# Merricx/zksnake

Measured on AMD Instinct MI355X. Metric: BN254 G1 MSM throughput, higher is better.
Workload: dtype u32 limbs (254-bit modular integers)

## Files before the change

### zksnake_amd/csrc/host.hip

```cpp
#include <dirent.h>
#include <unistd.h>
#include <cstring>
#include <map>
#include <mutex>
#include <vector>
#include "common.hip.h"
#include "codec.hip.h"

extern "C" void zk_ntt_free_cache(void);
extern "C" void zk_msm_free_all(void);
extern "C" void zk_ntt_stream_released(void* stream);

namespace zkmi {

static std::mutex g_cache_mutex;
static std::multimap<size_t, void*> g_cache_free;
static std::map<void*, size_t> g_cache_live;
static size_t g_cache_bytes = 0;
static const size_t CACHE_BUDGET = 6ull << 30;
static const size_t CACHE_MAX_BLOCK = 2ull << 30;

int dev_alloc_cached(void** p, size_t bytes) {
    if (bytes == 0) bytes = 1;
    {
        std::lock_guard<std::mutex> lock(g_cache_mutex);
        auto it = g_cache_free.find(bytes);
        if (it != g_cache_free.end()) {
            *p = it->second;
            g_cache_free.erase(it);
            g_cache_bytes -= bytes;
            g_cache_live[*p] = bytes;
            return ZK_OK;
        }
    }
    hipError_t e = hipMalloc(p, bytes);
    if (e != hipSuccess) {
        dev_cache_release();
        e = hipMalloc(p, bytes);
    }
    if (e != hipSuccess) return fail(ZK_ERR_HIP, std::string("hipMalloc(") + std::to_string(bytes) + " bytes): " + hipGetErrorString(e));
    std::lock_guard<std::mutex> lock(g_cache_mutex);
    g_cache_live[*p] = bytes;
    return ZK_OK;
}

void dev_free_cached(void* p) {
    if (!p) return;
    size_t bytes = 0;
    {
        std::lock_guard<std::mutex> lock(g_cache_mutex);
        auto it = g_cache_live.find(p);
        if (it != g_cache_live.end()) {
            bytes = it->second;
            g_cache_live.erase(it);
            if (bytes <= CACHE_MAX_BLOCK && g_cache_bytes + bytes <= CACHE_BUDGET) {
                g_cache_free.emplace(bytes, p);
                g_cache_bytes += bytes;
                return;
            }
        }
    }
    (void)hipFree(p);
}

static std::vector<hipStream_t> g_stream_pool[2];
static std::multimap<size_t, void*> g_pinned_free;
static std::map<void*, size_t> g_pinned_live;

void dev_cache_release() {
    std::lock_guard<std::mutex> lock(g_cache_mutex);
    for (auto& kv : g_cache_free) (void)hipFree(kv.second);
    g_cache_free.clear();
    g_cache_bytes = 0;
    for (auto& pool : g_stream_pool) {
        for (hipStream_t st : pool) (void)hipStreamDestroy(st);
        pool.clear();
    }
    for (auto& kv : g_pinned_free) (void)hipHostFree(kv.second);
    g_pinned_free.clear();
}

int stream_acquire(bool high_priority, hipStream_t* out) {
    {
        std::lock_guard<std::mutex> lock(g_cache_mutex);
        auto& pool = g_stream_pool[high_priority ? 1 : 0];
        if (!pool.empty()) {
            *out = pool.back();
            pool.pop_back();
            return ZK_OK;
        }
    }
    int lo = 0, hi = 0;
    ZK_HIP(hipDeviceGetStreamPriorityRange(&lo, &hi));
    ZK_HIP(hipStreamCreateWithPriority(out, hipStreamDefault, high_priority ? hi : lo));
    return ZK_OK;
}

void stream_release(bool high_priority, hipStream_t st) {
    if (!st) return;
    std::lock_guard<std::mutex> lock(g_cache_mutex);
    auto& pool = g_stream_pool[high_priority ? 1 : 0];
    if (pool.size() < 32) pool.push_back(st);
    else (void)hipStreamDestroy(st);
}

int pinned_alloc_cached(void** p, size_t bytes) {
    {
        std::lock_guard<std::mutex> lock(g_cache_mutex);
        auto it = g_pinned_free.find(bytes);
        if (it != g_pinned_free.end()) {
            *p = it->second;
            g_pinned_free.erase(it);
            g_pinned_live[*p] = bytes;
            return ZK_OK;
        }
    }
    ZK_HIP(hipHostMalloc(p, bytes));
    std::lock_guard<std::mutex> lock(g_cache_mutex);
    g_pinned_live[*p] = bytes;
    return ZK_OK;
}

void pinned_free_cached(void* p) {
    if (!p) return;
    std::lock_guard<std::mutex> lock(g_cache_mutex);
    auto it = g_pinned_live.find(p);
    if (it != g_pinned_live.end() && g_pinned_free.size() < 64 && it->second <= (1u << 20)) {
        g_pinned_free.emplace(it->second, p);
        g_pinned_live.erase(it);
        return;
    }
    if (it != g_pinned_live.end()) g_pinned_live.erase(it);
    (void)hipHostFree(p);
}


template <class G>
static Affine<typename G::F> load_point(const uint64_t* src) {
    typedef typename G::F F;
    const uint32_t* w = reinterpret_cast<const uint32_t*>(src);
    Affine<F> p;
    p.x = F::from_canonical(w);
    p.y = F::from_canonical(w + F::LIMBS);
    return p;
}

template <class G>
static void store_point(uint64_t* dst, const Affine<typename G::F>& p) {
    typedef typename G::F F;
    uint32_t* w = reinterpret_cast<uint32_t*>(dst);
    F::to_canonical(w, p.x);
    F::to_canonical(w + F::LIMBS, p.y);
}

template <class G>
static Affine<typename G::HostF> load_point64(const uint64_t* src) {
    typedef typename G::HostF HF;
    const uint32_t* w = reinterpret_cast<const uint32_t*>(src);
    return {HF::from_canonical(w), HF::from_canonical(w + HF::LIMBS)};
}
template <class G>
static void store_point64(uint64_t* dst, const Affine<typename G::HostF>& p) {
    G::HostF::affine_to_canonical(p, dst);
}

template <class G>
static bool point_on_curve(const Affine<typename G::F>& p) {
    typedef typename G::F F;
    typename F::T b = F::from_canonical(CurveConsts<G>::b());
    return aff_on_curve<F>(p, b);
}

template <class FrP>
static void reduce_scalar(uint32_t* k, const uint64_t* scalar) {
    memcpy(k, scalar, FrP::W * 4);
    for (int r = 0; r < 10; ++r) {
        uint32_t t[FrP::W];
        if (fp_sub_mod_raw<FrP>(t, k)) break;
        memcpy(k, t, sizeof(t));
    }
}


template <class G>
static int compress_impl(const uint64_t* a, uint8_t* out) {
    int code = point_encode<G>(reinterpret_cast<const uint32_t*>(a), out);
    return code ? fail(ZK_ERR_POINT, codec_message(code)) : ZK_OK;
}

template <class G>
static int decompress_impl(const uint8_t* in, uint64_t* out) {
    int code = point_decode<G>(in, reinterpret_cast<uint32_t*>(out));
    return code ? fail(ZK_ERR_POINT, codec_message(code)) : ZK_OK;
}


template <class P>
static Fp<P> fr_root(uint64_t n) {
    int log_n = log2_u64(n);
    Fp<P> w = fp_const<P>(P::ROOT);
    for (int k = 0; k < P::TWO_ADICITY - log_n; ++k) w = fp_sqr<P>(w);
    return w;
}

template <class P>
static int lagrange_impl(uint64_t n_in, const uint64_t* tau_c, uint64_t* out) {
    uint64_t n = next_pow2_u64(n_in == 0 ? 1 : n_in);
    int log_n = log2_u64(n);
    if (log_n > P::TWO_ADICITY) return fail(ZK_ERR_DOMAIN, "Domain size is too large");
    Fp<P> tau = fp_from_canonical<P>(reinterpret_cast<const uint32_t*>(tau_c));
    Fp<P> w = fr_root<P>(n);
    Fp<P> tn = tau;
    for (int k = 0; k < log_n; ++k) tn = fp_sqr<P>(tn);
    Fp<P> z = fp_sub<P>(tn, fp_one<P>());
    uint32_t* o = reinterpret_cast<uint32_t*>(out);
    if (fp_is_zero<P>(z)) {
        Fp<P> cur = fp_one<P>();
        for (uint64_t i = 0; i < n; ++i) {
            Fp<P> v = fp_eq<P>(cur, tau) ? fp_one<P>() : fp_zero<P>();
            fp_to_canonical<P>(o + i * P::W, v);
            cur = fp_mul<P>(cur, w);
        }
        return ZK_OK;
    }
    uint32_t nn[P::W] = {0};
    nn[0] = (uint32_t)n;
    nn[1] = (uint32_t)(n >> 32);
    Fp<P> zn = fp_mul<P>(z, fp_inv<P>(fp_from_canonical<P>(nn)));
    std::vector<Fp<P>> den(n), pre(n), wi(n);
    Fp<P> cur = fp_one<P>(), run = fp_one<P>();
    for (uint64_t i = 0; i < n; ++i) {
        wi[i] = cur;
        den[i] = fp_sub<P>(tau, cur);
        pre[i] = run;
        run = fp_mul<P>(run, den[i]);
        cur = fp_mul<P>(cur, w);
    }
    Fp<P> inv = fp_inv<P>(run);
    for (uint64_t i = n; i-- > 0;) {
        Fp<P> di = fp_mul<P>(inv, pre[i]);
        inv = fp_mul<P>(inv, den[i]);
        Fp<P> l = fp_mul<P>(fp_mul<P>(zn, wi[i]), di);
        fp_to_canonical<P>(o + i * P::W, l);
    }
    return ZK_OK;
}

template <class P>
static int poly_eval_impl(uint64_t n, const uint64_t* coeffs, const uint64_t* x_c, uint64_t* out) {
    const uint32_t* c = reinterpret_cast<const uint32_t*>(coeffs);
    Fp<P> x = fp_from_canonical<P>(reinterpret_cast<const uint32_t*>(x_c));
    Fp<P> acc = fp_zero<P>();
    for (uint64_t i = n; i-- > 0;) acc = fp_add<P>(fp_mul<P>(acc, x), fp_from_canonical<P>(c + i * P::W));
    fp_to_canonical<P>(reinterpret_cast<uint32_t*>(out), acc);
    return ZK_OK;
}

template <class P>
static int poly_div_linear_impl(uint64_t n, const uint64_t* coeffs, const uint64_t* root_c, uint64_t* q, uint64_t* rem) {
    const uint32_t* c = reinterpret_cast<const uint32_t*>(coeffs);
    uint32_t* qo = reinterpret_cast<uint32_t*>(q);
    Fp<P> root = fp_from_canonical<P>(reinterpret_cast<const uint32_t*>(root_c));
    Fp<P> carry = fp_zero<P>();
    for (uint64_t i = n; i-- > 1;) {
        carry = fp_add<P>(fp_from_canonical<P>(c + i * P::W), fp_mul<P>(carry, root));
        fp_to_canonical<P>(qo + (i - 1) * P::W, carry);
    }
    Fp<P> r0 = n ? fp_add<P>(fp_from_canonical<P>(c), fp_mul<P>(carry, root)) : fp_zero<P>();
    fp_to_canonical<P>(reinterpret_cast<uint32_t*>(rem), r0);
    return ZK_OK;
}

template <class P>
static int grand_product_impl(uint64_t n, const uint64_t* num, const uint64_t* den, uint64_t* out) {
    const uint32_t* a = reinterpret_cast<const uint32_t*>(num);
    const uint32_t* b = reinterpret_cast<const uint32_t*>(den);
    uint32_t* o = reinterpret_cast<uint32_t*>(out);
    std::vector<Fp<P>> d(n), pre(n);
    Fp<P> run = fp_one<P>();
    for (uint64_t i = 0; i < n; ++i) {
        d[i] = fp_from_canonical<P>(b + i * P::W);
        if (fp_is_zero<P>(d[i])) return fail(ZK_ERR_ARG, "grand product: zero denominator");
        pre[i] = run;
        run = fp_mul<P>(run, d[i]);
    }
    Fp<P> inv = fp_inv<P>(run);
    for (uint64_t i = n; i-- > 0;) {
        Fp<P> di = fp_mul<P>(inv, pre[i]);
        inv = fp_mul<P>(inv, d[i]);
        d[i] = di;
    }
    Fp<P> acc = fp_one<P>();
    fp_to_canonical<P>(o, acc);
    for (uint64_t i = 0; i < n; ++i) {
        acc = fp_mul<P>(fp_mul<P>(acc, fp_from_canonical<P>(a + i * P::W)), d[i]);
        fp_to_canonical<P>(o + (i + 1) * P::W, acc);
    }
    return ZK_OK;
}

template <class P>
static int scale_add_impl(uint64_t n, uint64_t* acc, const uint64_t* x, const uint64_t* s_c) {
    uint32_t* a = reinterpret_cast<uint32_t*>(acc);
    const uint32_t* xs = reinterpret_cast<const uint32_t*>(x);
    Fp<P> s = fp_from_canonical<P>(reinterpret_cast<const uint32_t*>(s_c));
    for (uint64_t i = 0; i < n; ++i) {
        Fp<P> v = fp_add<P>(fp_from_canonical<P>(a + i * P::W), fp_mul<P>(s, fp_from_canonical<P>(xs + i * P::W)));
        fp_to_canonical<P>(a + i * P::W, v);
    }
    return ZK_OK;
}

static int g_device = -1;

constexpr int ZK_WANT_HW_QUEUES = 12;
static std::mutex g_queue_mu;
static int g_queue_status = -1, g_queue_count = 0;

static bool hip_runtime_started() {
    if (const char* t = getenv("ZKMI_TEST_RUNTIME_STARTED")) return atoi(t) != 0;
    DIR* d = opendir("/proc/self/fd");
    if (!d) return false;
    bool found = false;
    char path[64], target[256];
    while (struct dirent* e = readdir(d)) {
        if (e->d_name[0] == '.') continue;
        snprintf(path, sizeof(path), "/proc/self/fd/%s", e->d_name);
        const ssize_t k = readlink(path, target, sizeof(target) - 1);
        if (k <= 0) continue;
        target[k] = 0;
        if (strcmp(target, "/dev/kfd") == 0) { found = true; break; }
    }
    closedir(d);
    return found;
}

static int hw_queues_prepare(int* queues) {
    std::lock_guard<std::mutex> lock(g_queue_mu);
    if (g_queue_status < 0) {
        const bool started = hip_runtime_started();
        const char* env = getenv("GPU_MAX_HW_QUEUES");
        if (env && *env) {
            g_queue_count = atoi(env);
            const char* ours = getenv("ZKMI_HW_QUEUES_SET_BY_LIBRARY");
            g_queue_status = (ours && *ours == '1' && g_queue_count == ZK_WANT_HW_QUEUES) ? ZK_QUEUES_SET_BY_LIBRARY : ZK_QUEUES_CALLER;
        } else if (!started) {
            char v[16];
            snprintf(v, sizeof(v), "%d", ZK_WANT_HW_QUEUES);
            setenv("GPU_MAX_HW_QUEUES", v, 0);
            setenv("ZKMI_HW_QUEUES_SET_BY_LIBRARY", "1", 1);
            g_queue_count = ZK_WANT_HW_QUEUES;
            g_queue_status = ZK_QUEUES_SET_BY_LIBRARY;
        } else {
            g_queue_count = 0;
            g_queue_status = ZK_QUEUES_TOO_LATE;
        }
    }
    if (queues) *queues = g_queue_count;
    return g_queue_status;
}

__global__ void spin_kernel(uint64_t ticks) {
    const uint64_t t0 = wall_clock64();
    while (wall_clock64() - t0 < ticks) {}
}

}

using namespace zkmi;

extern "C" {

int zk_device_count(void) {
    int n = 0;
    if (hipGetDeviceCount(&n) != hipSuccess) return 0;
    return n;
}

int zk_hw_queues_prepare(int* queues) { return hw_queues_prepare(queues); }

int zk_init(int device) {
    (void)hw_queues_prepare(nullptr);
    int n = zk_device_count();
    if (n <= 0) return fail(ZK_ERR_HIP, "no HIP device visible: libzkmi has no CPU fallback");
    if (device < 0 || device >= n) return fail(ZK_ERR_ARG, "device index out of range");
    ZK_HIP(hipSetDevice(device));
    g_device = device;
    return ZK_OK;
}

int zk_init_ex(int device, int* queue_status, int* queues) {
    const int st = hw_queues_prepare(queues);
    if (queue_status) *queue_status = st;
    return zk_init(device);
}

int zk_debug_spin_dev(void* stream, uint64_t microseconds) {
    hipLaunchKernelGGL(spin_kernel, dim3(1), dim3(64), 0, (hipStream_t)stream, microseconds * 100ull);
    ZK_HIP(hipGetLastError());
    return ZK_OK;
}

int zk_shutdown(void) {
    zk_msm_free_all();
    zk_ntt_free_cache();
    dev_cache_release();
    return ZK_OK;
}

int zk_dev_alloc(uint64_t bytes, void** d_ptr) {
    return dev_alloc_cached(d_ptr, bytes ? bytes : 1);
}
int zk_dev_free(void* d_ptr) {
    ZK_HIP(hipDeviceSynchronize());
    dev_free_cached(d_ptr);
    return ZK_OK;
}
int zk_dev_upload(void* d_dst, const void* h_src, uint64_t bytes) {
    if (bytes) ZK_HIP(hipMemcpy(d_dst, h_src, bytes, hipMemcpyHostToDevice));
    return ZK_OK;
// ... 189 lines not shown
```

### zksnake_amd/csrc/msm_impl.hip.h

```cpp
#pragma once
#include <algorithm>
#include <chrono>
#include <memory>
#include <vector>
#include "common.hip.h"
#include "msm_plan.h"
#include "pair.hip.h"
#include "setup_impl.hip.h"
#include "codec.hip.h"
#include "glv_params.h"

#include "msm_common.hip.h"
#include "msm_accumulate.hip.h"
#include "msm_reduce.hip.h"
#include "msm_host_tail.h"

namespace zkmi {
using mem::DevBuf;

#if defined(ZK_GROUP) && (!defined(ZK_PART) || ZK_PART == 0)
extern template __global__ void accumulate_kernel<ZK_GROUP>(const uint32_t*, const uint32_t*, const uint32_t*, const uint32_t*, uint32_t, uint32_t, uint32_t, uint32_t*, uint32_t*);
extern template __global__ void accumulate_split_kernel<ZK_GROUP>(const uint32_t*, const uint32_t*, const uint32_t*, const uint32_t*, uint32_t, uint32_t, uint32_t, uint32_t*, uint32_t*);
extern template __global__ void bases_to_mont_kernel<ZK_GROUP>(const uint32_t*, uint64_t, uint32_t*, int);
extern template __global__ void combine_kernel<ZK_GROUP>(const uint32_t*, const uint32_t*, uint32_t, uint32_t, const uint32_t*, const uint32_t*, uint32_t*);
extern template __global__ void strided_sum_kernel<ZK_GROUP>(const uint32_t*, uint32_t*, SumJob, SumJob, uint32_t);
extern template __global__ void weighted_sum_kernel<ZK_GROUP>(const uint32_t*, uint32_t, uint32_t, const uint32_t*, uint32_t, uint32_t*);
ZK_SETUP_EXTERN_TEMPLATES(ZK_GROUP)
ZK_CODEC_EXTERN_TEMPLATES(ZK_GROUP)
#endif

#if !defined(ZK_PART) || ZK_PART == 0

template <class G>
static int precompute_table(uint32_t* table, uint64_t n, int c, int w_first, int w_count) {
    typedef typename G::F F;
    constexpr int AW = 2 * F::LIMBS, XW = 4 * F::LIMBS;
    if (w_first == 0 && w_count == 1) return ZK_OK;
    DevBuf temp_buf;
    ZK_HIP_RC(temp_buf.alloc(n * XW * 4));
    uint32_t* const temp = temp_buf.as();
    const unsigned blocks = (unsigned)((n + 255) / 256);
    const unsigned nblocks = (unsigned)((n + (uint64_t)NORM_THREADS * NORM_E - 1) / ((uint64_t)NORM_THREADS * NORM_E));
    hipLaunchKernelGGL(dbl_rows_kernel<G>, dim3(blocks), dim3(256), 0, 0, temp, n, c * w_first, (const uint32_t*)table);
    if (w_first > 0) hipLaunchKernelGGL(normalize_kernel<G>, dim3(nblocks), dim3(NORM_THREADS), 0, 0, temp, n, table, 0);
    for (int k = 1; k < w_count; ++k) {
        hipLaunchKernelGGL(dbl_rows_kernel<G>, dim3(blocks), dim3(256), 0, 0, temp, n, c, (const uint32_t*)nullptr);
        hipLaunchKernelGGL(normalize_kernel<G>, dim3(nblocks), dim3(NORM_THREADS), 0, 0, temp, n, table + (size_t)k * n * AW, 0);
    }
    ZK_HIP(hipGetLastError());
    ZK_HIP(hipDeviceSynchronize());
    return ZK_OK;
}

template <class G>
struct FixedTable {
    std::vector<uint64_t> base;
    DevBuf d_table;
    int nwin = 0;
    std::mutex mu;
    static FixedTable& get() {
        static FixedTable* const t = new FixedTable();
        return *t;
    }
    void release() {
        std::lock_guard<std::mutex> lock(mu);
        d_table.reset();
        base.clear();
    }
    int ensure(const uint64_t* base_limbs) {
        typedef typename G::F F;
        typedef typename G::Fr FrP;
        constexpr int AW = 2 * F::LIMBS, XW = 4 * F::LIMBS;
        const size_t words64 = AW / 2;
        if (d_table && base.size() == words64 && memcmp(base.data(), base_limbs, words64 * 8) == 0) return ZK_OK;
        d_table.reset();
        base.clear();
        nwin = (FrP::BITS + 1 + FIXED_C - 1) / FIXED_C;
        std::vector<uint32_t> wb((size_t)nwin * AW);
        {
            const uint32_t* w = reinterpret_cast<const uint32_t*>(base_limbs);
            Affine<F> g = {F::from_canonical(w), F::from_canonical(w + F::LIMBS)};
            XYZZ<F> acc = xyzz_from_affine<F>(g);
            for (int j = 0; j < nwin; ++j) {
                Affine<F> a = xyzz_to_affine<F>(acc);
                F::store(wb.data() + (size_t)j * AW, a.x);
                F::store(wb.data() + (size_t)j * AW + F::LIMBS, a.y);
                if (j + 1 < nwin) for (int k = 0; k < FIXED_C; ++k) acc = xyzz_dbl<F>(acc);
            }
        }
        const uint64_t rows = (uint64_t)nwin * FIXED_HALF;
        DevBuf table, d_wb, temp;
        ZK_HIP_RC(table.alloc(rows * AW * 4));
        ZK_HIP_RC(d_wb.alloc(wb.size() * 4));
        ZK_HIP_RC(temp.alloc(rows * XW * 4));
        ZK_HIP(hipMemcpy(d_wb.as(), wb.data(), wb.size() * 4, hipMemcpyHostToDevice));
        hipLaunchKernelGGL(fixed_table_kernel<G>, dim3((unsigned)((rows + 255) / 256)), dim3(256), 0, 0, d_wb.as(), nwin, temp.as());
        hipLaunchKernelGGL(normalize_kernel<G>, dim3((unsigned)((rows + (uint64_t)NORM_THREADS * NORM_E - 1) / ((uint64_t)NORM_THREADS * NORM_E))),
                           dim3(NORM_THREADS), 0, 0, temp.as(), rows, table.as(), 0);
        ZK_HIP(hipGetLastError());
        ZK_HIP(hipDeviceSynchronize());
        d_table = std::move(table);
        base.assign(base_limbs, base_limbs + words64);
        return ZK_OK;
    }
};

template <class G>
struct MsmPlan : MsmPlanBase {
    typedef typename G::F F;
    typedef typename G::Fr FrP;
    static constexpr int AW = 2 * F::LIMBS;
    static constexpr int XW = 4 * F::LIMBS;
    static constexpr uint64_t SEG_TARGET_LANES = 256ull * 1024;
    static constexpr int MAX_C = 20;
    bool wide = false;
    enum class Phase { All, SortOnly, Rest };
    enum class Run { Idle, Sorted, Pending };

    struct Work {
        DevBuf partials, buckets, rows, fin;
        DevBuf parts;
        hipEvent_t ev_acc0 = nullptr, ev_accs = nullptr, ev_acc1 = nullptr;
        bool acc_from_accs = false;
        hipEvent_t ev_release = nullptr;
        bool lent = false;
        uint32_t seg_len = 0;
        int w_first = 0, w_count = 0;
        uint32_t groups = 0;
    };

    uint64_t n = 0;
    uint64_t n_api = 0;
    bool glv = false;
    bool pre = false;
    int pw_first = 0, pw_count = 0;
    ReduceShape shape;
    Work ws;
    MsmFront front;
    std::shared_ptr<DevBuf> bases_block;
    uint32_t* d_bases = nullptr;
    uint32_t* h_final = nullptr;
    hipEvent_t ev_start = nullptr, ev_end = nullptr;

    ~MsmPlan() override {
        (void)hipDeviceSynchronize();
        pinned_free_cached(h_final);
        for (hipEvent_t e : {ws.ev_acc0, ws.ev_accs, ws.ev_acc1, ws.ev_release, ev_start, ev_end}) if (e) (void)hipEventDestroy(e);
        stream_release((create_flags & ZK_MSM_HIGH_PRIORITY) != 0, own_stream);
    }

    int init(uint64_t n_points, const void* bases, int bases_on_device, int flags, int window_bits, int win_first, int win_count,
             const MsmPlan* share = nullptr) {
        const bool trace = opt.trace_init;
        auto t_prev = std::chrono::steady_clock::now();
        auto mark = [&](const char* what) {
            if (!trace) return;
            auto now = std::chrono::steady_clock::now();
            fprintf(stderr, "[plan init] %-24s %8.1f us\n", what, std::chrono::duration<double, std::micro>(now - t_prev).count());
            t_prev = now;
        };
        create_flags = flags;
        seg_lanes_at_init = opt.segment_lanes ? opt.segment_lanes : SEG_TARGET_LANES;
        pre = (flags & ZK_MSM_PRECOMPUTE) != 0;
        if (n_points == 0 || n_points > (1ull << 26)) return fail(ZK_ERR_ARG, "MSM size must be in [1, 2^26]");
        const MsmLayout lay = msm_layout(FrP::BITS, GlvOf<G>::OK, n_points, flags, window_bits, win_count <= 0);
        glv = share ? share->glv : lay.glv;
        n_api = n_points;
        n = glv ? 2 * n_points : n_points;
        entries_per_window = n;
        c = lay.c;
        if (c < 2 || c > MAX_C) return fail(ZK_ERR_ARG, "window bits must be in [2, 20]");
        if (c > 16 && !pre) return fail(ZK_ERR_ARG, "windows wider than 16 bits need a fixed-base plan (ZK_MSM_PRECOMPUTE)");
        wide = c > 16;
        nwin = glv ? glv_window_count(c) : window_count(FrP::BITS + 1, c);
        if (win_count <= 0) { win_first = 0; win_count = nwin; }
        if (win_first < 0 || win_first + win_count > nwin) return fail(ZK_ERR_ARG, "window range out of bounds");
        pw_first = win_first;
        pw_count = win_count;
        if (!reduce_shape(c, wide, &shape)) return fail(ZK_ERR_ARG, "window too wide for the reduction stage");
        const uint64_t entries = (uint64_t)pw_count * n;
        if (entries > 0x7FFFFFFFull) return fail(ZK_ERR_ARG, "MSM too large");

        ZK_HIP_RC(stream_acquire((flags & ZK_MSM_HIGH_PRIORITY) != 0, &own_stream));
        if (share) {
            bases_block = share->bases_block;
            d_bases = share->d_bases;
        } else {
            bases_block = std::make_shared<DevBuf>();
            ZK_HIP_RC(bases_block->alloc((pre ? (uint64_t)pw_count : 1ull) * n * AW * 4));
            d_bases = bases_block->as();
            if (bases_on_device) {
                launch_bases_to_mont<G>((const uint32_t*)bases, n_api, d_bases, glv ? 1 : 0, nullptr);
            } else {
                DevBuf tmp;
                ZK_HIP_RC(tmp.alloc(n_api * AW * 4));
                ZK_HIP(hipMemcpy(tmp.as(), bases, n_api * AW * 4, hipMemcpyHostToDevice));
                launch_bases_to_mont<G>(tmp.as(), n_api, d_bases, glv ? 1 : 0, nullptr);
                ZK_HIP(hipDeviceSynchronize());
            }
            ZK_HIP(hipGetLastError());
            if (pre) {
                int rc = precompute_table<G>(d_bases, n, c, pw_first, pw_count);
                if (rc) return rc;
            }
        }
        mark("stream + bases");
        {
            FrontLayout fl;
            fl.c = c; fl.B = shape.B; fl.n = n; fl.n_api = n_api; fl.pre = pre; fl.wide = wide; fl.glv = glv ? &GlvOf<G>::P::K : nullptr;
            fl.pw_first = pw_first; fl.pw_count = pw_count; fl.nwin = nwin; fl.curve = G::CURVE;
            ZK_HIP_RC(front.init(fl, &opt));
        }
        const uint64_t max_sets = pre ? 1ull : (uint64_t)pw_count;
        ZK_HIP_RC(pinned_alloc_cached((void**)&h_final, (size_t)max_sets * shape.blocks() * 2 * XW * 4));
        mark("scalars/digits/pinned");
        ZK_HIP(hipEventCreateWithFlags(&ev_start, hipEventDisableSystemFence));
        ZK_HIP(hipEventCreate(&ev_end));
        {
            const uint64_t keys = max_sets * shape.B;
            const uint32_t seg_full = pick_seg_len(entries);
            const uint64_t max_segs = std::max<uint64_t>(entries / seg_full, std::min<uint64_t>(entries / 8, seg_lanes_at_init)) + keys + 8;
            ZK_HIP_RC(front.alloc_workspace());
            ZK_HIP_RC(ws.partials.alloc(max_segs * XW * 4));
            ZK_HIP_RC(ws.buckets.alloc(keys * XW * 4));
            ZK_HIP_RC(ws.rows.alloc(max_sets * (shape.R + shape.C) * XW * 4));
            if (reduce_parts_per_set(shape)) ZK_HIP_RC(ws.parts.alloc(max_sets * reduce_parts_per_set(shape) * XW * 4));
            ZK_HIP_RC(ws.fin.alloc(max_sets * shape.blocks() * 2 * XW * 4));
            for (hipEvent_t* e : {&ws.ev_acc0, &ws.ev_accs, &ws.ev_acc1, &ws.ev_release}) ZK_HIP(hipEventCreate(e));
        }
        mark("workspace + events");
        ZK_HIP_RC(front.set_kernel_attributes());
        ZK_HIP(weighted_sum_set_attributes<G>());
        mark("func attributes");
        ZK_HIP(hipDeviceSynchronize());
        mark("device sync");
        return ZK_OK;
    }

    uint32_t pick_seg_len(uint64_t entries) const {
        const uint64_t target = opt.segment_lanes ? opt.segment_lanes : SEG_TARGET_LANES;
        uint64_t sl = (entries + target - 1) / target;
        if (sl < 8) sl = 8;
        if (sl > 64) sl = 64;
        if (pre) {
            uint64_t per_bucket = entries / shape.B;
            uint64_t want = (per_bucket + 11) / 12;
            if (want > sl) sl = want;
            if (sl > 1024) sl = 1024;
        }
        return (uint32_t)sl;
    }


    bool split_pairs_on() const {
        if constexpr (AccumulateSplit<G>::ON) return opt.split_pairs < 0 ? AccumulateSplit<G>::DEFAULT : opt.split_pairs != 0;
        return false;
    }

    int stage_accumulate(uint32_t m, const SortedView& sv, hipStream_t st, bool prio_steps) {
        Work& l = ws;
        const uint32_t n_keys = l.groups * shape.B;
        const uint64_t lanes_needed = ((uint64_t)l.w_count * m + sv.seg_len - 1) / sv.seg_len;
        launch_accumulate<G>(split_pairs_on(), lanes_needed, d_bases, sv.sorted, sv.bstart, sv.sstart, n_keys, sv.seg_len, prio_steps ? 1u : 0u,
                             l.partials.as(), l.buckets.as(), st);
        ZK_HIP(hipEventRecord(l.ev_acc1, st));
        launch_combine<G>(l.partials.as(), sv.sstart, n_keys, sv.big_list, sv.big_count, l.buckets.as(), st);
        ZK_HIP(hipGetLastError());
        return ZK_OK;
    }

    int stage_reduce(hipStream_t st) {
        Work& l = ws;
        const uint32_t groups = l.groups;
        const ReducePlan plan = reduce_plan(shape, groups, opt.sum_one_step, opt.lanes_per_output);
        uint32_t* const row_sums = l.rows.as();
        const uint32_t* in = l.buckets.as();
        for (int k = 0; k < plan.steps; ++k) {
            uint32_t* const out = k + 1 < plan.steps ? l.parts.as() : row_sums;
            launch_strided_sum<G>(in, out, plan.step[k].rows, plan.step[k].cols, plan.step[k].lpo, st);
            in = out;
        }
        launch_weighted_sum<G>(row_sums, shape.R, groups, row_sums + (size_t)groups * shape.R * XW, shape.C, l.fin.as(), st);
        ZK_HIP(hipGetLastError());
        ZK_HIP(hipMemcpyAsync(h_final, l.fin.as(), (size_t)groups * shape.blocks() * 2 * XW * 4, hipMemcpyDeviceToHost, st));
        return ZK_OK;
    }

    int run_stages(uint32_t m, uint32_t dstride, hipStream_t st, const SortExport* borrowed = nullptr, Phase phase = Phase::All, hipEvent_t gate = nullptr) {
        Work& l = ws;
        int rc;
        const uint32_t seg_len = borrowed ? borrowed->view.seg_len : (phase == Phase::Rest ? l.seg_len : pick_seg_len((uint64_t)l.w_count * m));
        l.seg_len = seg_len;
        if (phase == Phase::Rest) {
        } else if (borrowed) {
            ZK_HIP(hipStreamWaitEvent(st, borrowed->sorted_ready, 0));
        } else if ((rc = front.sort(m, dstride, seg_len, l.w_first, l.w_count, l.groups, st))) {
            return rc;
        }
        const SortedView sv = borrowed ? borrowed->view : front.view();
        if (phase != Phase::Rest) ZK_HIP(hipEventRecord(l.ev_acc0, st));
        if (phase == Phase::SortOnly) return ZK_OK;
        if (gate) ZK_HIP(hipStreamWaitEvent(st, gate, 0));
        l.acc_from_accs = gate != nullptr || phase == Phase::Rest;
        if (l.acc_from_accs) ZK_HIP(hipEventRecord(l.ev_accs, st));
        const bool prio_steps = opt.priority_steps && phase == Phase::All && !gate && !borrowed;
        if ((rc = stage_accumulate(m, sv, st, prio_steps))) return rc;
        if (borrowed) ZK_HIP(hipEventRecord(borrowed->release, st));
        return stage_reduce(st);
    }

    int set_option(const char* name, int64_t value) override {
        std::lock_guard<std::mutex> lock(mu);
        if (in_flight()) return fail(ZK_ERR_ARG, "MSM plan has a run in flight: options change between runs");
        if (!strcmp(name, "segment_lanes")) {
            if (value < 64) return fail(ZK_ERR_ARG, "segment_lanes must be at least 64");
            if ((uint64_t)value > seg_lanes_at_init) return fail(ZK_ERR_ARG, "segment_lanes cannot exceed the value the plan was created with");
            opt.segment_lanes = (uint64_t)value;
        } else if (!strcmp(name, "sum_one_step")) {
            opt.sum_one_step = value != 0;
        } else if (!strcmp(name, "lanes_per_output")) {
            if (value != 0 && (value < 2 || value > 64 || (value & (value - 1)))) return fail(ZK_ERR_ARG, "lanes_per_output: 0 or a power of two in [2, 64]");
            opt.lanes_per_output = (uint32_t)value;
        } else if (!strcmp(name, "priority_steps")) {
            opt.priority_steps = value != 0;
        } else if (!strcmp(name, "split_pairs")) {
            if (value < -1 || value > 1) return fail(ZK_ERR_ARG, "split_pairs: -1 (the group's default), 0 or 1");
            if (value == 1 && !AccumulateSplit<G>::ON) return fail(ZK_ERR_ARG, "split_pairs: this group has no pair-split accumulate kernel (base-field groups)");
            opt.split_pairs = (int)value;
        } else if (!strcmp(name, "two_level_sort")) {
            if (value && !front.has_two_level_buffers()) return fail(ZK_ERR_ARG, "the plan was created without the buffers of the two-level sort");
            if (!value && wide) return fail(ZK_ERR_ARG, "windows wider than 16 bits exist in the two-level sort only");
            opt.two_level_sort = value != 0;
        } else {
            return fail(ZK_ERR_ARG, std::string("unknown or creation-time MSM option: ") + name);
        }
        return ZK_OK;
    }

    int debug_view(uint64_t* out, int cap) override {
        std::lock_guard<std::mutex> lock(mu);
        if (in_flight()) return fail(ZK_ERR_ARG, "MSM plan has a run in flight: the view is read between runs");
        if (!out || cap < ZK_MSM_VIEW_SLOTS) return fail(ZK_ERR_ARG, "zk_msm_plan_debug_view needs room for ZK_MSM_VIEW_SLOTS values");
        const SortedView own = front.view();
        const uint64_t v[ZK_MSM_VIEW_SLOTS] = {
            (uint64_t)(uintptr_t)front.digits_buf(), (uint64_t)(uintptr_t)d_bases, (uint64_t)(uintptr_t)own.sorted, (uint64_t)(uintptr_t)own.bstart,
            (uint64_t)(uintptr_t)own.sstart, (uint64_t)(uintptr_t)own.big_list, (uint64_t)(uintptr_t)own.big_count,
            (uint64_t)(uintptr_t)ws.partials.as(), (uint64_t)(uintptr_t)ws.buckets.as(),
            n, n_api, (uint64_t)c, (uint64_t)nwin, shape.B, glv ? 1u : 0u, pre ? 1u : 0u, wide ? 1u : 0u, (uint64_t)pw_first, (uint64_t)pw_count,
            (uint64_t)ws.w_first, (uint64_t)ws.w_count, ws.groups, ws.seg_len, q_m, front.view_dstride,
            (uint64_t)front.view_route, (uint64_t)front.view_fine_log, front.view_split_fine() ? 1u : 0u, split_pairs_on() ? 1u : 0u};
        for (int k = 0; k < ZK_MSM_VIEW_SLOTS; ++k) out[k] = v[k];
        return ZK_OK;
    }

    uint64_t seg_lanes_at_init = 0;
    int create_flags = 0;
    int clone(MsmPlanBase** out) override {
        MsmPlan* p = new MsmPlan();
        p->opt = opt;
        int rc = p->init(n_api, nullptr, 0, create_flags & ~ZK_MSM_HIGH_PRIORITY, c, pw_first, pw_count, this);
        if (rc) {
            delete p;
            return rc;
        }
        *out = p;
        return ZK_OK;
    }

    Run q_state = Run::Idle;
    int q_first = 0, q_count = 0;
    uint32_t q_m = 0;
    hipStream_t q_stream = nullptr;
    bool in_flight() const { return q_state != Run::Idle; }

    int begin_run(hipStream_t st, int w_first, int w_count, uint32_t m, uint32_t groups, const void* host_scalars = nullptr, size_t scalar_bytes = 0) {
        if (in_flight()) return fail(ZK_ERR_ARG, "MSM plan already has a run in flight: call zk_msm_plan_finish first");
        q_first = w_first; q_count = w_count; q_m = m; q_stream = st;
        if (ws.lent) {
            ZK_HIP(hipStreamWaitEvent(st, ws.ev_release, 0));
            ws.lent = false;
        }
        if (m == 0) return ZK_OK;
        if (host_scalars) ZK_HIP(hipMemcpyAsync(front.scalars_buf(), host_scalars, scalar_bytes, hipMemcpyHostToDevice, st));
        ZK_HIP(hipEventRecord(ev_start, st));
        ws.w_first = w_first;
        ws.w_count = w_count;
        ws.groups = groups;
        return ZK_OK;
    }

    int enqueue(uint64_t n_scalars, const void* scalars, int on_device, int w_first, int w_count, hipStream_t st) override {
        return enqueue_phase(n_scalars, scalars, on_device, w_first, w_count, st, Phase::All);
    }
    int enqueue_sort(uint64_t n_scalars, const void* scalars, int on_device, int w_first, int w_count, hipStream_t st) override {
        return enqueue_phase(n_scalars, scalars, on_device, w_first, w_count, st, Phase::SortOnly);
    }
    hipEvent_t accumulate_done_event() override { return ws.ev_acc1; }
    int enqueue_rest(MsmPlanBase* after) override {
        std::lock_guard<std::mutex> lock(mu);
        if (q_state != Run::Sorted) return fail(ZK_ERR_ARG, "zk_msm_plan_enqueue_rest without zk_msm_plan_enqueue_sort");
        q_state = Run::Idle;
        if (q_m > 0) {
            int rc = run_stages(q_m, (q_m + 7u) & ~7u, q_stream, nullptr, Phase::Rest, after ? after->accumulate_done_event() : nullptr);
            if (rc) return rc;
            ZK_HIP(hipEventRecord(ev_end, q_stream));
        }
        q_state = Run::Pending;
        return ZK_OK;
    }

    int enqueue_phase(uint64_t n_scalars, const void* scalars, int on_device, int w_first, int w_count, hipStream_t st, Phase phase) {
        std::lock_guard<std::mutex> lock(mu);
        if (n_scalars > n_api) return fail(ZK_ERR_LENGTH, "Number of points and scalars mismatch");
        if (w_count <= 0) { w_first = pw_first; w_count = pw_count; }
        if (w_first < pw_first || w_first + w_count > pw_first + pw_count)
            return fail(ZK_ERR_ARG, "window range out of bounds (the plan was created for windows [" + std::to_string(pw_first) + ", " +
                                        std::to_string(pw_first + pw_count) + "))");
        const uint32_t m_api = (uint32_t)n_scalars;
        const uint32_t m = glv ? 2 * m_api : m_api;
        int rc = begin_run(st, w_first, w_count, m, pre ? 1u : (uint32_t)w_count, on_device ? nullptr : scalars, (size_t)m_api * FrP::W * 4);
        if (rc) return rc;
        if (m > 0) {
            const uint32_t* sc = on_device ? (const uint32_t*)scalars : front.scalars_buf();
            if ((rc = front.digits(sc, m_api, w_first, w_count, st))) return rc;
            if ((rc = run_stages(m, (m + 7u) & ~7u, st, nullptr, phase))) return rc;
            if (phase == Phase::All) ZK_HIP(hipEventRecord(ev_end, st));
        }
        q_state = phase == Phase::SortOnly ? Run::Sorted : Run::Pending;
        return ZK_OK;
    }

    int cancel() override {
        std::lock_guard<std::mutex> lock(mu);
        if (in_flight() && q_stream) ZK_HIP(hipStreamSynchronize(q_stream));
        q_state = Run::Idle;
        return ZK_OK;
    }

    int export_sort(SortExport* out) override {
        std::lock_guard<std::mutex> lock(mu);
        if (!in_flight() || q_m == 0) return fail(ZK_ERR_ARG, "the lending plan has no run in flight");
        out->view = front.view();
        out->view.seg_len = ws.seg_len;
        out->n = n; out->m = q_m; out->groups = ws.groups;
        out->c = c; out->nwin = nwin; out->w_first = q_first; out->w_count = q_count;
        out->pw_first = pw_first; out->pw_count = pw_count; out->scalar_bits = FrP::BITS; out->pre = pre; out->glv = glv;
        out->endo = glv ? G::ENDO_ID : 0;
        out->sorted_ready = ws.ev_acc0;
        out->release = ws.ev_release;
        ws.lent = true;
        return ZK_OK;
    }

    int enqueue_shared(MsmPlanBase* lender, hipStream_t st) override {
        SortExport ex;
        int rc = lender->export_sort(&ex);
        if (rc) return rc;
        std::lock_guard<std::mutex> lock(mu);
        if (ex.n != n || ex.c != c || ex.nwin != nwin || ex.pre != pre || ex.glv != glv || ex.endo != (glv ? G::ENDO_ID : 0) || ex.scalar_bits != FrP::BITS ||
            ex.pw_first != pw_first || ex.pw_count != pw_count)
            return fail(ZK_ERR_ARG, "plans differ in size, window layout or mode: the sort cannot be shared");
        if ((rc = begin_run(st, ex.w_first, ex.w_count, ex.m, ex.groups))) return rc;
        if ((rc = run_stages(ex.m, (ex.m + 7u) & ~7u, st, &ex))) return rc;
        ZK_HIP(hipEventRecord(ev_end, st));
        q_state = Run::Pending;
        return ZK_OK;
    }

    int finish(uint64_t* out) override {
        std::lock_guard<std::mutex> lock(mu);
        if (q_state == Run::Sorted) return fail(ZK_ERR_ARG, "zk_msm_plan_finish before zk_msm_plan_enqueue_rest");
        if (q_state != Run::Pending) return fail(ZK_ERR_ARG, "zk_msm_plan_finish without a pending run");
        q_state = Run::Idle;
        if (q_m > 0) ZK_HIP(hipEventSynchronize(ev_end));
        const auto tail_t0 = std::chrono::steady_clock::now();
        int rc = msm_host_tail<G>(h_final, q_m > 0 ? ws.groups : 0u, shape, c, q_first, pre, out);
        if (rc || q_m == 0) return rc;
        timings[3] = std::chrono::duration<float, std::milli>(std::chrono::steady_clock::now() - tail_t0).count();
        auto elapsed = [](hipEvent_t from, hipEvent_t to) {
            float t = 0;
            return hipEventElapsedTime(&t, from, to) == hipSuccess ? t : 0.0f;
        };
        timings[0] = elapsed(ev_start, ws.ev_acc0);
        timings[1] = elapsed(ws.acc_from_accs ? ws.ev_accs : ws.ev_acc0, ws.ev_acc1);
        timings[2] = elapsed(ws.ev_acc1, ev_end);
        float t = 0;
        timings[4] = hipEventElapsedTime(&t, ev_start, ev_end) == hipSuccess ? t + timings[3] : 0.0f;
        return ZK_OK;
    }
};

constexpr uint64_t FIXED_BASE_MIN = 2048;

template <class G>
static int batch_mul_impl(uint64_t n, const uint64_t* scalars, const uint64_t* bases, int broadcast, uint64_t* out) {
    typedef typename G::F F;
    typedef typename G::Fr FrP;
    constexpr int AW = 2 * F::LIMBS, XW = 4 * F::LIMBS;
    if (n == 0) return ZK_OK;
    DevBuf ds, db, dout, temp;
    const bool fixed = broadcast && n >= FIXED_BASE_MIN;
    uint64_t nb = broadcast ? 1 : n;
    ZK_HIP_RC(ds.alloc(n * FrP::W * 4));
    ZK_HIP_RC(temp.alloc(n * XW * 4));
    ZK_HIP_RC(dout.alloc(n * AW * 4));
    ZK_HIP(hipMemcpy(ds.as(), scalars, n * FrP::W * 4, hipMemcpyHostToDevice));
    if (fixed) {
        FixedTable<G>& ft = FixedTable<G>::get();
        std::lock_guard<std::mutex> lock(ft.mu);
        ZK_HIP_RC(ft.ensure(bases));
        FixedBias bias;
        memset(&bias, 0, sizeof(bias));
        for (int j = 0; j < ft.nwin; ++j) {
            int bit = j * FIXED_C + (FIXED_C - 1);
            bias.v[bit >> 5] |= 1u << (bit & 31);
        }
        hipLaunchKernelGGL(fixed_mul_kernel<G>, dim3((unsigned)((n + 255) / 256)), dim3(256), 0, 0, ds.as(), n, ft.d_table.as(), ft.nwin, bias, temp.as());
        ZK_HIP(hipDeviceSynchronize());
    } else {
        ZK_HIP_RC(db.alloc(nb * AW * 4));
        ZK_HIP(hipMemcpy(db.as(), bases, nb * AW * 4, hipMemcpyHostToDevice));
        hipLaunchKernelGGL(varbase_mul_kernel<G>, dim3((unsigned)((n + 127) / 128)), dim3(128), 0, 0, ds.as(), db.as(), broadcast, n, temp.as());
    }
    hipLaunchKernelGGL(normalize_kernel<G>, dim3((unsigned)((n + (uint64_t)NORM_THREADS * NORM_E - 1) / ((uint64_t)NORM_THREADS * NORM_E))),
                       dim3(NORM_THREADS), 0, 0, temp.as(), n, dout.as(), 1);
    ZK_HIP(hipGetLastError());
    ZK_HIP(hipMemcpy(out, dout.as(), n * AW * 4, hipMemcpyDeviceToHost));
    return ZK_OK;
}

template <class G>
static int codec_impl(uint64_t n, const void* in, void* out, int to_bytes, uint64_t* bad_index) {
    typedef typename G::F F;
    constexpr size_t ROW = (size_t)2 * F::LIMBS * 4, ENC = CodecLayout<G>::TOTAL;
    if (n == 0) return ZK_OK;
    const size_t in_bytes = n * (to_bytes ? ROW : ENC), out_bytes = n * (to_bytes ? ENC : ROW);
    DevBuf din, dout, derr;
    ZK_HIP_RC(din.alloc(in_bytes));
    ZK_HIP_RC(dout.alloc(out_bytes));
    ZK_HIP_RC(derr.alloc(8));
    unsigned long long first = ~0ull;
    ZK_HIP(hipMemcpy(din.as(), in, in_bytes, hipMemcpyHostToDevice));
    ZK_HIP(hipMemcpy(derr.as(), &first, 8, hipMemcpyHostToDevice));
    const dim3 grid((unsigned)((n + 127) / 128)), block(128);
    if (to_bytes) hipLaunchKernelGGL(points_encode_kernel<G>, grid, block, 0, 0, din.as<const uint32_t>(), n, dout.as<uint8_t>(), derr.as<unsigned long long>());
    else hipLaunchKernelGGL(points_decode_kernel<G>, grid, block, 0, 0, din.as<const uint8_t>(), n, dout.as(), derr.as<unsigned long long>());
    ZK_HIP(hipGetLastError());
    ZK_HIP(hipMemcpy(&first, derr.as(), 8, hipMemcpyDeviceToHost));
    if (first != ~0ull) {
        if (bad_index) *bad_index = (uint64_t)(first >> 8);
        return fail(ZK_ERR_POINT, codec_message((int)(first & 0xFF)));
    }
    ZK_HIP(hipMemcpy(out, dout.as(), out_bytes, hipMemcpyDeviceToHost));
    return ZK_OK;
}


#endif

}
```

### zksnake_amd/csrc/msm_reduce.hip.h

```cpp
#pragma once
#include "msm_common.hip.h"
#include "msm_reduce_plan.h"

namespace zkmi {

constexpr int COMBINE_THREADS = 256;
constexpr uint32_t COMBINE_WAVE_BLOCKS = 128, COMBINE_BIG_BLOCKS = 64;

template <class G>
__global__ __launch_bounds__(COMBINE_THREADS) void combine_kernel(const uint32_t* __restrict__ partials,
                                                                  const uint32_t* __restrict__ run_start, uint32_t n_keys,
                                                                  uint32_t small_blocks, const uint32_t* __restrict__ big_list,
                                                                  const uint32_t* __restrict__ big_count,
                                                                  uint32_t* __restrict__ buckets) {
    typedef typename G::F F;
    constexpr int XW = 4 * F::LIMBS;
    constexpr int HW = HalfRegs<F>::COUNT;
    __shared__ uint32_t sh[COMBINE_THREADS * HW];
    const bool odd = (threadIdx.x & 1) != 0;
    if (blockIdx.x < small_blocks) {
        const uint32_t key = (blockIdx.x * COMBINE_THREADS + threadIdx.x) >> 1;
        if (key >= n_keys) return;
        const uint32_t s0 = run_start[key], s1 = run_start[key + 1];
        if (s1 - s0 == 1 || s1 - s0 > COMBINE_SMALL_MAX) return;
        HalfPt<F> acc = half_inf<F>();
        if (s1 > s0) {
            acc = half_load<F>(partials + (size_t)s0 * XW, odd);
            HalfPt<F> cur = s0 + 1 < s1 ? half_load<F>(partials + (size_t)(s0 + 1) * XW, odd) : half_inf<F>();
            for (uint32_t r = s0 + 1; r < s1; ++r) {
                HalfPt<F> nxt = r + 1 < s1 ? half_load<F>(partials + (size_t)(r + 1) * XW, odd) : half_inf<F>();
                acc = pair_add<F>(acc, cur, odd);
                cur = nxt;
            }
        }
        half_store<F>(buckets + (size_t)key * XW, odd, acc);
    } else if (blockIdx.x < small_blocks + COMBINE_WAVE_BLOCKS) {
        const uint32_t count = big_count[0];
        const uint32_t lane = threadIdx.x & 63, pair = lane >> 1;
        const uint32_t wave = ((blockIdx.x - small_blocks) * COMBINE_THREADS + threadIdx.x) >> 6;
        const uint32_t n_waves = (COMBINE_WAVE_BLOCKS * COMBINE_THREADS) >> 6;
        for (uint32_t b = wave; b < count; b += n_waves) {
            const uint32_t key = big_list[b];
            const uint32_t s0 = run_start[key], s1 = run_start[key + 1];
            HalfPt<F> v = half_inf<F>();
            for (uint32_t r = s0 + pair; r < s1; r += 32) v = pair_add<F>(v, half_load<F>(partials + (size_t)r * XW, odd), odd);
            for (int m = 32; m >= 2; m >>= 1) v = pair_add<F>(v, half_shfl_xor<F>(v, m), odd);
            if (lane < 2) half_store<F>(buckets + (size_t)key * XW, odd, v);
        }
    } else {
        const uint32_t count = big_count[1];
        const uint32_t j = threadIdx.x, pair = j >> 1;
        for (uint32_t b = blockIdx.x - small_blocks - COMBINE_WAVE_BLOCKS; b < count; b += COMBINE_BIG_BLOCKS) {
            const uint32_t key = big_list[n_keys - 1 - b];
            const uint32_t s0 = run_start[key], s1 = run_start[key + 1];
            HalfPt<F> v = half_inf<F>();
            for (uint32_t r = s0 + pair; r < s1; r += COMBINE_THREADS / 2) v = pair_add<F>(v, half_load<F>(partials + (size_t)r * XW, odd), odd);
            for (uint32_t off = COMBINE_THREADS / 4; off >= 1; off >>= 1) {
                half_lds_put<F>(sh, COMBINE_THREADS, j, v);
                __syncthreads();
                if (pair < off) v = pair_add<F>(v, half_lds_get<F>(sh, COMBINE_THREADS, j + 2 * off), odd);
                __syncthreads();
            }
            if (j < 2) half_store<F>(buckets + (size_t)key * XW, odd, v);
        }
    }
}


template <class G>
__global__ __launch_bounds__(256) void strided_sum_kernel(const uint32_t* __restrict__ in, uint32_t* __restrict__ out,
                                                          SumJob j0, SumJob j1, uint32_t lpo) {
    typedef typename G::F F;
    constexpr int XW = 4 * F::LIMBS;
    const uint32_t gid = blockIdx.x * blockDim.x + threadIdx.x;
    uint32_t o = gid / lpo;
    const uint32_t sub = gid % lpo;
    const bool odd = (sub & 1) != 0;
    const uint32_t pair = sub >> 1, n_pairs = lpo >> 1;
    SumJob job = j0;
    if (o >= j0.n_out) {
        o -= j0.n_out;
        job = j1;
    }
    const bool live = o < job.n_out;
    const uint32_t x = live ? o % job.per_group : 0;
    size_t base = live ? (size_t)job.in_offset + (size_t)(o / job.per_group) * job.group_stride + (size_t)(x / job.split) * job.outer + (size_t)(x % job.split) * job.outer2 : 0;
    HalfPt<F> acc = half_inf<F>();
    if (live && pair < job.count) {
        HalfPt<F> cur = half_load<F>(in + (base + (size_t)pair * job.inner) * XW, odd);
        for (uint32_t j = pair; j < job.count; j += n_pairs) {
            const uint32_t jn = j + n_pairs < job.count ? j + n_pairs : j;
            HalfPt<F> nxt = half_load<F>(in + (base + (size_t)jn * job.inner) * XW, odd);
            acc = pair_add<F>(acc, cur, odd);
            cur = nxt;
        }
    }
    for (uint32_t m = lpo >> 1; m >= 2; m >>= 1) {
        HalfPt<F> other = half_shfl_xor<F>(acc, (int)m);
        acc = pair_add<F>(acc, other, odd);
    }
    if (live && sub < 2) half_store<F>(out + ((size_t)job.out_offset + o) * XW, odd, acc);
}

constexpr int HS_THREADS = 2 * WS_BLOCK;
template <class G>
__global__ __launch_bounds__(HS_THREADS) void weighted_sum_kernel(const uint32_t* __restrict__ in0, uint32_t m0, uint32_t n0,
                                                                  const uint32_t* __restrict__ in1, uint32_t m1,
                                                                  uint32_t* __restrict__ out) {
    typedef typename G::F F;
    constexpr int XW = 4 * F::LIMBS;
    extern __shared__ uint32_t sh[];
    const uint32_t tid = threadIdx.x, pj = tid >> 1;
    const bool odd = (tid & 1) != 0;
    const uint32_t bpa0 = (m0 + WS_BLOCK - 1) / WS_BLOCK, bpa1 = (m1 + WS_BLOCK - 1) / WS_BLOCK;
    const bool first = blockIdx.x < n0 * bpa0;
    const uint32_t rel = first ? blockIdx.x : blockIdx.x - n0 * bpa0;
    const uint32_t bpa = first ? bpa0 : bpa1, ma = first ? m0 : m1;
    const uint32_t arr_i = rel / bpa, blk = rel % bpa;
    const uint32_t m = min((uint32_t)WS_BLOCK, ma - blk * WS_BLOCK);
    const uint32_t* arr = (first ? in0 : in1) + ((size_t)arr_i * ma + (size_t)blk * WS_BLOCK) * XW;
    HalfPt<F> v = pj < m ? half_load<F>(arr + (size_t)pj * XW, odd) : half_inf<F>();
    for (uint32_t off = 1; off < m; off <<= 1) {
        half_lds_put<F>(sh, HS_THREADS, tid, v);
        __syncthreads();
        if (pj + off < m) {
            HalfPt<F> o = half_lds_get<F>(sh, HS_THREADS, tid + 2 * off);
            v = pair_add<F>(v, o, odd);
        }
        __syncthreads();
    }
    if (pj == 0) half_store<F>(out + ((size_t)blockIdx.x * 2 + 1) * XW, odd, v);
    if (pj == 0 || pj >= m) v = half_inf<F>();
    uint32_t top = 1;
    while (top < m) top <<= 1;
    for (uint32_t off = top / 2; off >= 1; off >>= 1) {
        half_lds_put<F>(sh, HS_THREADS, tid, v);
        __syncthreads();
        if (pj < off) {
            HalfPt<F> o = half_lds_get<F>(sh, HS_THREADS, tid + 2 * off);
            v = pair_add<F>(v, o, odd);
        }
        __syncthreads();
    }
    if (pj == 0) half_store<F>(out + (size_t)blockIdx.x * 2 * XW, odd, v);
}


template <class G>
inline void launch_combine(const uint32_t* partials, const uint32_t* run_start, uint32_t n_keys, const uint32_t* big_list,
                           const uint32_t* big_count, uint32_t* buckets, hipStream_t st) {
    const uint32_t small_blocks = (2 * n_keys + COMBINE_THREADS - 1) / COMBINE_THREADS;
    hipLaunchKernelGGL(combine_kernel<G>, dim3(small_blocks + COMBINE_WAVE_BLOCKS + COMBINE_BIG_BLOCKS), dim3(COMBINE_THREADS), 0, st,
                       partials, run_start, n_keys, small_blocks, big_list, big_count, buckets);
}

template <class G>
inline void launch_strided_sum(const uint32_t* in, uint32_t* out, const SumJob& j0, const SumJob& j1, uint32_t lpo, hipStream_t st) {
    hipLaunchKernelGGL(strided_sum_kernel<G>, dim3((unsigned)((((uint64_t)j0.n_out + j1.n_out) * lpo + 255) / 256)), dim3(256), 0, st,
                       in, out, j0, j1, lpo);
}

template <class G>
inline hipError_t weighted_sum_set_attributes() {
    return hipFuncSetAttribute((const void*)weighted_sum_kernel<G>, hipFuncAttributeMaxDynamicSharedMemorySize,
                               (int)(HalfRegs<typename G::F>::COUNT * HS_THREADS * 4));
}

template <class G>
inline void launch_weighted_sum(const uint32_t* in0, uint32_t m0, uint32_t n0, const uint32_t* in1, uint32_t m1, uint32_t* out, hipStream_t st) {
    const uint32_t blocks = n0 * ((m0 + WS_BLOCK - 1) / WS_BLOCK + (m1 + WS_BLOCK - 1) / WS_BLOCK);
    hipLaunchKernelGGL(weighted_sum_kernel<G>, dim3(blocks), dim3(HS_THREADS), (size_t)HalfRegs<typename G::F>::COUNT * HS_THREADS * 4, st,
                       in0, m0, n0, in1, m1, out);
}

}
```

Before: 694.3.

## Write MSM final sums to mapped host memory and compact small-bucket combine work

After: 701.1, median of 4. About the same (+1.0%).

```diff
diff --git a/zksnake_amd/csrc/host.hip b/zksnake_amd/csrc/host.hip
--- a/zksnake_amd/csrc/host.hip
+++ b/zksnake_amd/csrc/host.hip
@@ -115,7 +115,7 @@
             return ZK_OK;
         }
     }
-    ZK_HIP(hipHostMalloc(p, bytes));
+    ZK_HIP(hipHostMalloc(p, bytes, hipHostMallocMapped | hipHostMallocCoherent));
     std::lock_guard<std::mutex> lock(g_cache_mutex);
     g_pinned_live[*p] = bytes;
     return ZK_OK;
diff --git a/zksnake_amd/csrc/msm_impl.hip.h b/zksnake_amd/csrc/msm_impl.hip.h
--- a/zksnake_amd/csrc/msm_impl.hip.h
+++ b/zksnake_amd/csrc/msm_impl.hip.h
@@ -118,7 +118,7 @@
     enum class Run { Idle, Sorted, Pending };
 
     struct Work {
-        DevBuf partials, buckets, rows, fin;
+        DevBuf partials, buckets, rows;
         DevBuf parts;
         hipEvent_t ev_acc0 = nullptr, ev_accs = nullptr, ev_acc1 = nullptr;
         bool acc_from_accs = false;
@@ -140,6 +140,7 @@
     std::shared_ptr<DevBuf> bases_block;
     uint32_t* d_bases = nullptr;
     uint32_t* h_final = nullptr;
+    uint32_t* d_final = nullptr;
     hipEvent_t ev_start = nullptr, ev_end = nullptr;
 
     ~MsmPlan() override {
@@ -213,6 +214,7 @@
         }
         const uint64_t max_sets = pre ? 1ull : (uint64_t)pw_count;
         ZK_HIP_RC(pinned_alloc_cached((void**)&h_final, (size_t)max_sets * shape.blocks() * 2 * XW * 4));
+        ZK_HIP(hipHostGetDevicePointer((void**)&d_final, h_final, 0));
         mark("scalars/digits/pinned");
         ZK_HIP(hipEventCreateWithFlags(&ev_start, hipEventDisableSystemFence));
         ZK_HIP(hipEventCreate(&ev_end));
@@ -225,7 +227,6 @@
             ZK_HIP_RC(ws.buckets.alloc(keys * XW * 4));
             ZK_HIP_RC(ws.rows.alloc(max_sets * (shape.R + shape.C) * XW * 4));
             if (reduce_parts_per_set(shape)) ZK_HIP_RC(ws.parts.alloc(max_sets * reduce_parts_per_set(shape) * XW * 4));
-            ZK_HIP_RC(ws.fin.alloc(max_sets * shape.blocks() * 2 * XW * 4));
             for (hipEvent_t* e : {&ws.ev_acc0, &ws.ev_accs, &ws.ev_acc1, &ws.ev_release}) ZK_HIP(hipEventCreate(e));
         }
         mark("workspace + events");
@@ -280,9 +281,8 @@
             launch_strided_sum<G>(in, out, plan.step[k].rows, plan.step[k].cols, plan.step[k].lpo, st);
             in = out;
         }
-        launch_weighted_sum<G>(row_sums, shape.R, groups, row_sums + (size_t)groups * shape.R * XW, shape.C, l.fin.as(), st);
+        launch_weighted_sum<G>(row_sums, shape.R, groups, row_sums + (size_t)groups * shape.R * XW, shape.C, d_final, st);
         ZK_HIP(hipGetLastError());
-        ZK_HIP(hipMemcpyAsync(h_final, l.fin.as(), (size_t)groups * shape.blocks() * 2 * XW * 4, hipMemcpyDeviceToHost, st));
         return ZK_OK;
     }
 
diff --git a/zksnake_amd/csrc/msm_reduce.hip.h b/zksnake_amd/csrc/msm_reduce.hip.h
--- a/zksnake_amd/csrc/msm_reduce.hip.h
+++ b/zksnake_amd/csrc/msm_reduce.hip.h
@@ -5,6 +5,7 @@
 namespace zkmi {
 
 constexpr int COMBINE_THREADS = 256;
+constexpr int COMBINE_PAIRS = COMBINE_THREADS / 2, COMBINE_WAVES = COMBINE_THREADS / 64;
 constexpr uint32_t COMBINE_WAVE_BLOCKS = 128, COMBINE_BIG_BLOCKS = 64;
 
 template <class G>
@@ -17,23 +18,59 @@
     constexpr int XW = 4 * F::LIMBS;
     constexpr int HW = HalfRegs<F>::COUNT;
     __shared__ uint32_t sh[COMBINE_THREADS * HW];
+    __shared__ uint32_t q_key[COMBINE_PAIRS], q_next[COMBINE_PAIRS], q_end[COMBINE_PAIRS], q_count[COMBINE_WAVES];
     const bool odd = (threadIdx.x & 1) != 0;
     if (blockIdx.x < small_blocks) {
+        const uint32_t lane = threadIdx.x & 63, wave = threadIdx.x >> 6;
         const uint32_t key = (blockIdx.x * COMBINE_THREADS + threadIdx.x) >> 1;
-        if (key >= n_keys) return;
-        const uint32_t s0 = run_start[key], s1 = run_start[key + 1];
-        if (s1 - s0 == 1 || s1 - s0 > COMBINE_SMALL_MAX) return;
-        HalfPt<F> acc = half_inf<F>();
-        if (s1 > s0) {
-            acc = half_load<F>(partials + (size_t)s0 * XW, odd);
-            HalfPt<F> cur = s0 + 1 < s1 ? half_load<F>(partials + (size_t)(s0 + 1) * XW, odd) : half_inf<F>();
-            for (uint32_t r = s0 + 1; r < s1; ++r) {
-                HalfPt<F> nxt = r + 1 < s1 ? half_load<F>(partials + (size_t)(r + 1) * XW, odd) : half_inf<F>();
+        const bool in_range = key < n_keys;
+        const uint32_t s0 = in_range ? run_start[key] : 0, s1 = in_range ? run_start[key + 1] : 0;
+        const uint32_t runs = s1 - s0;
+        const bool mine = in_range && runs != 1 && runs <= COMBINE_SMALL_MAX;
+        const bool more = mine && runs > 2;
+        const uint64_t handing = __ballot(more);
+        if (lane == 0) q_count[wave] = (uint32_t)__popcll(handing) >> 1;
+        if (mine) {
+            HalfPt<F> acc = half_inf<F>();
+            if (runs >= 2) {
+                const HalfPt<F> first = half_load<F>(partials + (size_t)s0 * XW, odd);
+                acc = pair_add<F>(first, half_load<F>(partials + (size_t)(s0 + 1) * XW, odd), odd);
+            }
+            if (!more) half_store<F>(buckets + (size_t)key * XW, odd, acc);
+            if (more) {
+                const uint32_t slot = wave * 32 + ((uint32_t)__popcll(handing & ((1ull << (lane & ~1u)) - 1)) >> 1);
+                half_lds_put<F>(sh, COMBINE_THREADS, 2 * slot + (odd ? 1u : 0u), acc);
+                if (!odd) {
+                    q_key[slot] = key;
+                    q_next[slot] = s0 + 2;
+                    q_end[slot] = s1;
+                }
+            }
+        }
+        __syncthreads();
+        uint32_t g = threadIdx.x >> 1, src = 0, total = 0;
+        bool found = false;
+#pragma unroll
+        for (uint32_t w = 0; w < COMBINE_WAVES; ++w) {
+            const uint32_t cnt = q_count[w];
+            if (!found && g < total + cnt) {
+                found = true;
+                src = w * 32 + (g - total);
+            }
+            total += cnt;
+        }
+        if (found) {
+            HalfPt<F> acc = half_lds_get<F>(sh, COMBINE_THREADS, 2 * src + (odd ? 1u : 0u));
+            const uint32_t k2 = q_key[src], e = q_end[src];
+            uint32_t r = q_next[src];
+            HalfPt<F> cur = half_load<F>(partials + (size_t)r * XW, odd);
+            for (; r < e; ++r) {
+                HalfPt<F> nxt = r + 1 < e ? half_load<F>(partials + (size_t)(r + 1) * XW, odd) : half_inf<F>();
                 acc = pair_add<F>(acc, cur, odd);
                 cur = nxt;
             }
-        }
-        half_store<F>(buckets + (size_t)key * XW, odd, acc);
+            half_store<F>(buckets + (size_t)k2 * XW, odd, acc);
+        }
     } else if (blockIdx.x < small_blocks + COMBINE_WAVE_BLOCKS) {
         const uint32_t count = big_count[0];
         const uint32_t lane = threadIdx.x & 63, pair = lane >> 1;
```
